# Maaz77/Head-Pose-Estimation-Model

Hardware: AMD Instinct MI355X
Metric: images/sec (train+infer) on 96×96 feature maps; yaw/pitch/roll MAE vs ref (higher is better)
Workload: dtype fp32; 1 GPU; Model-96 create_model(num_filters=360, dropout=0, l2=0.1) training, legacy Adam lr 2.8e-4, 96x96 feature maps (configs[3] per GPU: 512 images per rank); global_batch=512, per_gpu_batch=512, positions_per_image=9216, channels=96, parallelism=dp1

## Files before the change

head-pose-estimation-model_amd/csrc/hpe_mlp2.hip:

```cpp
#include <hip/hip_runtime.h>
#include <stdint.h>
#include <stdlib.h>

#include "hpe_common.h"
#include "hpe_dev.h"

#ifdef MLP2_BIG
#define MLP2_NS mlp2_big
#else
#define MLP2_NS mlp2_small
#endif
#define MLP2_BIG_ROWS (1 << 15)
namespace MLP2_NS {

#define MLP2_MAXW 12
#ifndef MLP2_BAR1_SKIP
#define MLP2_BAR1_SKIP 1
#endif
#ifndef MLP2_W88
#define MLP2_W88 2
#endif
#define MLP2_XS 100
#define MLP2_XF (32 * MLP2_XS)
#define MLP2_LAB 128
#define MLP2_RED 32
#define MLP2_FS 104
#define MLP2_IMG (3 * 32 * MLP2_FS)
#define MLP2_A1W (15 * 68 + 64)
#define MLP2_PRE_HALVES (2 * MLP2_IMG)

struct E2 {
  int act, drop;
  uint32_t thr;
  float keep;
};

struct TileImg {
  int img0, rem0, P;
  template <bool P32 = false>
  __device__ __forceinline__ int of(int r) const {
    const int t = rem0 + r;
    if (P32) return img0 + (t >= P ? 1 : 0);
    return img0 + (P >= 32 ? (t >= P ? 1 : 0) : (P == 1 ? t : t / P));
  }
  __device__ __forceinline__ void advance(int dq, int dr) {
    img0 += dq;
    rem0 += dr;
    if (rem0 >= P) { rem0 -= P; ++img0; }
  }
};

__device__ __forceinline__ float e_fwd(const E2& e, uint64_t seed, int64_t img, int ch, float z) {
  float a = act_f(e.act, z);
  if (e.drop >= 0) a = drop_hash(seed, e.drop, (uint64_t)img, ch) >= e.thr ? a / e.keep : 0.f;
  return a;
}

__device__ __forceinline__ float e_bwd(const E2& e, uint64_t seed, int64_t img, int ch, float g, float val) {
  if (e.drop >= 0) {
    if (drop_hash(seed, e.drop, (uint64_t)img, ch) < e.thr) return 0.f;
    g = g / e.keep;
    val = val * e.keep;
  }
  return e.act == ACT_LINEAR ? g : g * act_grad(e.act, val, 0.f);
}

__device__ __forceinline__ void stage_tile(const Args& args, float* xs, float* lab, int64_t row0,
                                           const TileImg& ti, int wave, int NCB, int lane, int Cin,
                                           bool labels, int XS = MLP2_XS) {
  const int64_t rem = args.nrows - 1 - row0;
  const int last = rem < 31 ? (int)rem : 31;
  const int P = args.P;
  const int q = Cin >> 2;
  if (!args.idx && P >= 32) {
    if (labels && wave == 0) {
#pragma unroll
      for (int pc = 0; pc < 2; ++pc) {
        const int slot = pc * 64 + lane;
        const int r = min(slot >> 2, last), j = min(slot & 3, 2);
        glds4(args.ytrue + (int64_t)ti.of(r) * 3 + j, lds_addr(lab + pc * 64));
      }
    }
    for (int r = wave; r < 32; r += NCB) {
      const int64_t srow = row0 + min(r, last);
      if (lane < q) glds16(args.x + srow * Cin + 4 * lane, lds_addr(xs + r * XS));
    }
    return;
  }
  const int lr = min(lane & 31, last);
  const int limg = ti.of(lr);
  const int lpos = (int)(row0 + lr - (int64_t)limg * P);
  const int lsrc = args.idx ? args.idx[limg] : limg;
  __builtin_amdgcn_s_waitcnt(0x0F70);
  if (labels && wave == 0) {
#pragma unroll
    for (int pc = 0; pc < 2; ++pc) {
      const int slot = pc * 64 + lane;
      const int r = min(slot >> 2, last), j = min(slot & 3, 2);
      const int64_t src = __shfl(lsrc, r, 64);
      glds4(args.ytrue + src * 3 + j, lds_addr(lab + pc * 64));
    }
  }
  for (int r = wave; r < 32; r += NCB) {
    const int rr = min(r, last);
    const int64_t srow = (int64_t)__builtin_amdgcn_readlane(lsrc, rr) * P +
                         __builtin_amdgcn_readlane(lpos, rr);
    if (lane < q) glds16(args.x + srow * Cin + 4 * lane, lds_addr(xs + r * XS));
  }
}

__device__ __forceinline__ int lane_now() {
  int l;
  asm volatile("v_mbcnt_lo_u32_b32 %0, -1, 0\n\tv_mbcnt_hi_u32_b32 %0, -1, %0" : "=v"(l));
  return l;
}

__device__ __forceinline__ void stage_contig(const Args& args, float* xs, float* lab, const float* tp,
                                             int64_t row0, const TileImg& ti, int wave, int NCB, int Cin,
                                             bool labels) {
  const int lane = lane_now();
  const int64_t rem = args.nrows - 1 - row0;
  const int last = rem < 31 ? (int)rem : 31;
  if (labels && wave == 0) {
    const float* yp = args.ytrue + (int64_t)ti.img0 * 3;
#pragma unroll
    for (int pc = 0; pc < 2; ++pc) {
      const int slot = pc * 64 + lane;
      const int r = min(slot >> 2, last), j = min(slot & 3, 2);
      glds4(yp + (ti.rem0 + r >= ti.P ? 3 + j : j), lds_addr(lab + pc * 64));
    }
  }
  const int q = Cin >> 2;
  for (int r = wave; r < 32; r += NCB)
    if (lane < q) glds16(tp + min(r, last) * Cin + 4 * lane, lds_addr(xs + r * MLP2_XS));
}

typedef _Float16 h4 __attribute__((ext_vector_type(4)));

typedef __fp16 fp16x4 __attribute__((__vector_size__(4 * sizeof(__fp16))));

template <int KH>
__device__ __forceinline__ int img_pos(int c) {
  if (KH == 48) return c;
  return c < KH ? c : min(c + 48 - KH, 92);
}
__device__ __forceinline__ h8 tr_read8(const _Float16* p) {
  typedef __attribute__((address_space(3))) fp16x4* lp;
  const fp16x4 a = __builtin_amdgcn_ds_read_tr16_b64_v4f16((lp)(p));
  const fp16x4 b = __builtin_amdgcn_ds_read_tr16_b64_v4f16((lp)(p + 8 * MLP2_FS));
  return __builtin_shufflevector(__builtin_bit_cast(h4, a), __builtin_bit_cast(h4, b), 0, 1, 2, 3, 4, 5, 6, 7);
}
__device__ __forceinline__ constexpr int a1_row(int g) { return 68 * (g ^ ((g >> 1) & 4)); }
#define MLP2_X_LIMIT (65520.f / SPLIT_C)
template <int KH>
__device__ __forceinline__ bool presplit_tile(const float* xs, _Float16* xf, int tid, int NT) {
  bool out = false;
  for (int i = tid; i < 32 * 12; i += NT) {
    const int r = i / 12, rem = i - r * 12, h = rem >= 6 ? 1 : 0, m0 = 8 * (rem - 6 * h);
    const float* s = xs + r * MLP2_XS + KH * h + m0;
    const f32x4 z = {0.f, 0.f, 0.f, 0.f};
    const f32x4 a = *(const f32x4*)(s), b = m0 + 4 < KH ? *(const f32x4*)(s + 4) : z;
    const f32x8 v = {a.x, a.y, a.z, a.w, b.x, b.y, b.z, b.w};
#pragma unroll
    for (int j = 0; j < 8; ++j) out |= !(fabsf(v[j]) < MLP2_X_LIMIT);
    const SplitD d8 = split_d8(v);
    _Float16* d = xf + r * MLP2_FS + 48 * h + m0;
    *(h8*)(d) = d8.ch;
    *(h8*)(d + 32 * MLP2_FS) = d8.cl;
    *(h8*)(d + 64 * MLP2_FS) = d8.h;
  }
  return out;
}

template <int KH, int ACT1, bool DROP, int NWM, bool SPLIT, bool CONTIG = false>
__global__ void __launch_bounds__(NWM * 64) __attribute__((amdgpu_waves_per_eu(NWM == MLP2_MAXW || ACT1 < 0 ? 1 : MLP2_W88, 8))) mlp2_kernel(Args args) {
  static_assert(!CONTIG || (SPLIT && NWM == MLP2_MAXW), "CONTIG is an instantiation of the pre-split kernel");
  if (!SPLIT && args.guard && __hip_atomic_load(args.guard, __ATOMIC_RELAXED, __HIP_MEMORY_SCOPE_AGENT) != args.epoch) return;
#ifdef MLP2_STAMPS
  const uint64_t rt0 = __builtin_amdgcn_s_memrealtime();
#endif
  extern __shared__ __attribute__((aligned(16))) float lds[];
  constexpr int NKB = (2 * KH + 31) / 32;
  constexpr int T = 32;
  constexpr bool PRE = SPLIT && NWM == MLP2_MAXW;
  constexpr int NXB = PRE ? 1 : 2;
  constexpr bool LEAN = PRE && ACT1 >= 0;
  constexpr bool PAD1 = true;
  constexpr int A1S = MLP2_A1W;
  constexpr int HS = NWM == MLP2_MAXW ? 4 : 3;
  const int* prog = args.prog;
  const int* o = prog + prog[H_OPS_OFF];
  const int mode = prog[H_MODE];
  const bool train = mode == MODE_TRAIN;
  const int Cin = o[O_K], F = o[O_N], NCB = o[O_MODE];
  const int wave = __builtin_amdgcn_readfirstlane(threadIdx.x >> 6);
  const int lane = threadIdx.x & 63, half = lane >> 5, l32 = lane & 31;
  const int NT = blockDim.x;
  const int n = wave * 32 + l32;
  const bool nok = n < F;
  const int NPR = NWM == MLP2_MAXW ? MLP2_MAXW : NCB;
  float* xbuf = lds;
  float* lbuf = xbuf + NXB * MLP2_XF;
  float* part = lbuf + 2 * MLP2_LAB;
  float* dz2 = part + NPR * T * 4;
  float* a1s = dz2 + T * 4;
  float* w2t = a1s + NCB * A1S;
  float* b2t = w2t + NCB * 128;
  float* hacc = b2t + 4;
  float* red = hacc + NCB * 64 * HS;
  float* colt = red + MLP2_RED;
  _Float16* xfb = (_Float16*)(colt + NCB * 128);

  E2 e1 = {o[O_EACT], o[O_EDROP], (uint32_t)o[O_ETHR], __int_as_float(o[O_EKEEP])};
  E2 e2 = {o[O_AUX2], o[O_TBASE], (uint32_t)o[O_TCOUNT], __int_as_float(o[O_F0])};
  const float inv_keep1 = 1.f / e1.keep;
  const float* W1 = args.params + o[O_W];
  const float* W2 = args.params + o[O_AUX0];

  const int64_t nrows = args.nrows;
  const int64_t ntiles = (nrows + T - 1) / T;
  const int P = args.P;
  const bool labels = mode != MODE_FWD;
  const int S = gridDim.x * T, dq = S / P, dr = S - dq * P;
  TileImg ti;
  ti.P = P;
  ti.img0 = (int)(blockIdx.x * T / P);
  ti.rem0 = (int)(blockIdx.x * T - ti.img0 * P);
  const float* xnext = CONTIG ? args.x + (int64_t)blockIdx.x * T * Cin : nullptr;
  const int64_t xstep = CONTIG ? (int64_t)gridDim.x * T * Cin : 0;
  if (blockIdx.x < ntiles) {
    if constexpr (CONTIG) stage_contig(args, xbuf, lbuf, xnext, (int64_t)blockIdx.x * T, ti, wave, NCB, Cin, labels);
    else stage_tile(args, xbuf, lbuf, (int64_t)blockIdx.x * T, ti, wave, NCB, lane, Cin, labels);
  }
  xnext += xstep;
  const int nc = min(n, F - 1);
  const float w2a = W2[nc * 3], w2b = W2[nc * 3 + 1], w2c = W2[nc * 3 + 2];
  const int o_bias = __builtin_amdgcn_readfirstlane(o[O_BIAS]), o_aux1 = __builtin_amdgcn_readfirstlane(o[O_AUX1]);
  const float b1r = args.params[max(o_bias, 0) + nc];
  float w2r[2];
#pragma unroll
  for (int t = 0; t < 2; ++t) {
    const int i = threadIdx.x + t * NT, nn = i >> 2, j = i & 3;
    w2r[t] = W2[min(nn, F - 1) * 3 + min(j, 2)];
  }
  const float b2r = args.params[max(o_aux1, 0) + min((int)threadIdx.x & 3, 2)];

  float wreg[SPLIT ? 1 : KH];
  SplitW wsp[SPLIT ? 6 : 1];
  float inv1 = 1.f, s2 = 1.f;
  bool wbad = false;
  if constexpr (SPLIT) {
    f32x8 v[6];
#pragma unroll
    for (int s = 0; s < 6; ++s) {
#pragma unroll
      for (int j = 0; j < 8; ++j) {
        const int k = half * KH + 8 * s + j;
        v[s][j] = 8 * s + j < KH ? W1[(size_t)min(k, Cin - 1) * F + nc] : 0.f;
      }
    }
    __builtin_amdgcn_sched_barrier(0);
    float mx = 0.f;
#pragma unroll
    for (int s = 0; s < 6; ++s) {
#pragma unroll
      for (int j = 0; j < 8; ++j) {
        const int k = half * KH + 8 * s + j;
        v[s][j] = (k < Cin && nok) ? v[s][j] : 0.f;
        mx = fmaxf(mx, fabsf(v[s][j]));
      }
    }
    mx = fmaxf(mx, __shfl_xor(mx, 32, 64));
    const float s1 = pow2_scale(mx, 13);
    inv1 = SPLIT_INV_C / s1;
#pragma unroll
    for (int s = 0; s < 6; ++s) {
      const f32x8 vs = v[s] * s1;
      wsp[s] = split_w8(vs);
      if (PRE) {
#pragma unroll
        for (int j = 0; j < 8; ++j) wbad |= !(fabsf(vs[j]) < 65520.f);
      }
    }
    s2 = pow2_scale(nok ? fmaxf(fmaxf(fabsf(w2a), fabsf(w2b)), fabsf(w2c)) : 0.f, 2);
  } else {
#pragma unroll
    for (int m = 0; m < KH; ++m) {
      const int k = half * KH + m;
      const float wv = W1[(size_t)min(k, Cin - 1) * F + nc];
      wreg[m] = (k < Cin && nok) ? wv : 0.f;
    }
  }
  bool bad = PRE && wbad && blockIdx.x < ntiles;
  {
    const float b1 = (nok && o_bias >= 0) ? b1r : 0.f;
    if (half == 0) *(f32x4*)(colt + n * 4) = f32x4{inv1, b1, s2, 0.f};
  }
#pragma unroll
  for (int t = 0; t < 2; ++t) {
    const int i = threadIdx.x + t * NT, nn = i >> 2, j = i & 3;
    if (i < NCB * 128) w2t[i] = (nn < F && j < 3) ? w2r[t] : 0.f;
  }
  if (threadIdx.x < 4) b2t[threadIdx.x] = (threadIdx.x < 3 && o_aux1 >= 0) ? b2r : 0.f;
  for (int i = threadIdx.x; i < NT * HS; i += NT) hacc[i] = 0.f;

  f32x16 dw[NKB];
#pragma unroll
  for (int s = 0; s < NKB; ++s) dw[s] = f32x16{};
  float dw2[3] = {0.f, 0.f, 0.f};
  float db1 = 0.f;

  const int NT3 = (NT / 3) * 3;

  for (int i = threadIdx.x; i < NXB * 32 * 16; i += NT) {
    const int r = i >> 4, c = Cin + (i & 15);
    if (c < 96) xbuf[r * MLP2_XS + c] = 0.f;
  }
  for (int i = NCB * T * 4 + threadIdx.x; i < NPR * T * 4; i += NT) part[i] = 0.f;
  __syncthreads();
  if constexpr (PRE) {
    asm volatile("s_waitcnt vmcnt(0)" ::: "memory");
    bar_lds();
    const bool xbad = presplit_tile<KH>(xbuf, xfb, threadIdx.x, NT);
    bad |= xbad && blockIdx.x < ntiles;
  }
  int buf = 0;
#ifdef MLP2_STAMPS
  uint32_t ph[9] = {};
  uint64_t tprev = __builtin_amdgcn_s_memtime();
  const uint64_t rt1 = __builtin_amdgcn_s_memrealtime();
#define STAMP(i) do { const uint64_t t_ = __builtin_amdgcn_s_memtime(); ph[i] += (uint32_t)(t_ - tprev); tprev = t_; } while (0)
#else
#define STAMP(i) do {} while (0)
#endif
  for (int tile = blockIdx.x; tile < (int)ntiles; tile += gridDim.x, buf ^= 1, ti.advance(dq, dr)) {
    const int tlane = PRE ? lane_now() : lane, thalf = tlane >> 5, tl32 = tlane & 31;
    const int tcol = wave * 32 + tl32;
    const bool tok = tcol < F;
    const int64_t row0 = (int64_t)tile * T;
    const float* xs = xbuf + (PRE ? 0 : buf) * MLP2_XF;
    const float* lab = lbuf + buf * MLP2_LAB;
    if constexpr (!PRE) asm volatile("s_waitcnt vmcnt(0)" ::: "memory");
    STAMP(0);
    if (!(MLP2_BAR1_SKIP && PRE && tile != (int)blockIdx.x)) bar_lds();
    STAMP(1);
    if (tile + gridDim.x < ntiles) {
      TileImg tn = ti;
      tn.advance(dq, dr);
      if constexpr (CONTIG) {
        stage_contig(args, xbuf, lbuf + (buf ^ 1) * MLP2_LAB, xnext, (int64_t)(tile + gridDim.x) * T, tn,
                     wave, NCB, Cin, labels);
        xnext += xstep;
      } else {
        stage_tile(args, xbuf + (PRE ? 0 : (buf ^ 1)) * MLP2_XF, lbuf + (buf ^ 1) * MLP2_LAB,
                   (int64_t)(tile + gridDim.x) * T, tn, wave, NCB, tlane, Cin, labels);
      }
    }

    STAMP(2);
    uint32_t dmask = 0;
    {
      const float* ap = xs + tl32 * MLP2_XS + thalf * KH;
      f32x16 acc = {};
      if constexpr (PRE) {
        const _Float16* fp = xfb + buf * MLP2_IMG + tl32 * MLP2_FS + 48 * thalf;
        auto frag = [&](int s) {
          return SplitD{*(const h8*)(fp + 8 * s), *(const h8*)(fp + 32 * MLP2_FS + 8 * s),
                        *(const h8*)(fp + 64 * MLP2_FS + 8 * s)};
        };
        SplitD xd = frag(0);
#pragma unroll
        for (int s = 0; s < 6; ++s) {
          SplitD xn = xd;
          if (s + 1 < 6) xn = frag(s + 1);
          __builtin_amdgcn_sched_barrier(0);
          acc = mfma3_dw(xd, wsp[s], acc);
          xd = xn;
        }
        STAMP(3);
      } else if constexpr (SPLIT) {
#pragma unroll
        for (int s = 0; s < 6; ++s) {
          const f32x4 a0 = *(const f32x4*)(ap + 8 * s), a1 = *(const f32x4*)(ap + 8 * s + 4);
          acc = mfma3_dw(split_d8(f32x8{a0.x, a0.y, a0.z, a0.w, a1.x, a1.y, a1.z, a1.w}), wsp[s], acc);
          __builtin_amdgcn_sched_barrier(0);
        }
        bad |= !(fabsf(sum16(acc)) <= 3.0e38f);
      } else {
        f32x4 an = *(const f32x4*)(ap);
#pragma unroll
        for (int m = 0; m < KH; m += 4) {
          const f32x4 a = an;
          if (m + 4 < KH) an = *(const f32x4*)(ap + m + 4);
          acc = __builtin_amdgcn_mfma_f32_32x32x2f32(a.x, wreg[m + 0], acc, 0, 0, 0);
          acc = __builtin_amdgcn_mfma_f32_32x32x2f32(a.y, wreg[m + 1], acc, 0, 0, 0);
          acc = __builtin_amdgcn_mfma_f32_32x32x2f32(a.z, wreg[m + 2], acc, 0, 0, 0);
          acc = __builtin_amdgcn_mfma_f32_32x32x2f32(a.w, wreg[m + 3], acc, 0, 0, 0);
          __builtin_amdgcn_sched_barrier(0);
        }
      }
      if (DROP) {
        if (CONTIG || P >= 32) {
          const bool k0 = drop_hash(args.seed, e1.drop, (uint64_t)(ti.img0 + args.img_off), tcol) >= e1.thr;
          const bool k1 = drop_hash(args.seed, e1.drop, (uint64_t)(ti.img0 + 1 + args.img_off), tcol) >= e1.thr;
#pragma unroll
          for (int g = 0; g < 16; ++g) {
            const int r = (g & 3) + 8 * (g >> 2) + 4 * thalf;
            dmask |= (ti.rem0 + r >= P ? k1 : k0) ? (1u << g) : 0u;
          }
        } else {
#pragma unroll
          for (int g = 0; g < 16; ++g) {
            const int r = (g & 3) + 8 * (g >> 2) + 4 * thalf;
            dmask |= drop_hash(args.seed, e1.drop, (uint64_t)(ti.of(r) + args.img_off), tcol) >= e1.thr
                         ? (1u << g) : 0u;
          }
        }
      }
      const f32x4 cs = *(const f32x4*)(colt + tcol * 4);
#pragma unroll
      for (int g = 0; g < 16; ++g) {
        float z = act1_f<ACT1, SPLIT>(e1.act, SPLIT ? fmaf(acc[g], cs.x, cs.y) : acc[g] + cs.y);
        if (DROP) z = (dmask >> g) & 1u ? z * inv_keep1 : 0.f;
        acc[g] = LEAN || tok ? z : 0.f;
      }
#pragma unroll
      for (int g = 0; g < 16; ++g) a1s[wave * A1S + (PAD1 ? a1_row(g) : 64 * g) + tlane] = acc[g];
      __builtin_amdgcn_fence(__ATOMIC_RELEASE, "wavefront");
      __builtin_amdgcn_wave_barrier();
      __builtin_amdgcn_fence(__ATOMIC_ACQUIRE, "wavefront");
      {
        const int r = tl32, hh = (r >> 2) & 1, gr = (r & 3) + 4 * (r >> 3);
        const float* ar = a1s + wave * A1S + (PAD1 ? a1_row(gr) : 64 * gr) + hh * 32 + 16 * thalf;
        const float* wr = w2t + (wave * 32 + 16 * thalf) * 4;
        float s0 = 0.f, s1 = 0.f, s2 = 0.f;
#pragma unroll
        for (int i = 0; i < 16; i += 4) {
          const f32x4 av = *(const f32x4*)(ar + i);
#pragma unroll
          for (int e = 0; e < 4; ++e) {
            const f32x4 w = *(const f32x4*)(wr + (i + e) * 4);
            s0 = fmaf(av[e], w.x, s0);
            s1 = fmaf(av[e], w.y, s1);
            s2 = fmaf(av[e], w.z, s2);
          }
        }
        s0 += __shfl_xor(s0, 32, 64);
        s1 += __shfl_xor(s1, 32, 64);
        s2 += __shfl_xor(s2, 32, 64);
        if (thalf == 0) *(f32x4*)(part + (wave * T + r) * 4) = f32x4{s0, s1, s2, 0.f};
      }
    }
    STAMP(4);
    if constexpr (PRE) asm volatile("s_waitcnt vmcnt(0)" ::: "memory");
    bar_lds();
    STAMP(5);
    if constexpr (PRE) {
      if (wave >= 2 && tile + gridDim.x < ntiles)
        bad |= presplit_tile<KH>(xbuf, xfb + (buf ^ 1) * MLP2_IMG, threadIdx.x - 128, NT - 128);
    }

    auto head_item = [&](int it) {
      const int r = it / 3, j = it - r * 3;
      const int64_t R = row0 + r;
      float z = b2t[j];
      float pv[MLP2_MAXW];
#pragma unroll
      for (int w = 0; w < MLP2_MAXW; ++w) pv[w] = NWM == MLP2_MAXW || w < NCB ? part[(w * T + r) * 4 + j] : 0.f;
      float lv = 0.f, ha0 = 0.f, ha1 = 0.f, ha2 = 0.f;
      if (mode != MODE_FWD) {
        lv = lab[r * 4 + j];
        ha0 = hacc[threadIdx.x * HS + 0];
        ha1 = hacc[threadIdx.x * HS + 1];
        ha2 = hacc[threadIdx.x * HS + 2];
      }
#pragma unroll
      for (int w = 0; w < MLP2_MAXW; ++w) z += pv[w];
      const bool d2 = ACT1 < 0 || __builtin_expect(e2.drop >= 0, 0);
      int64_t img = 0;
      bool k2 = true;
      if (d2) {
        img = ti.of<CONTIG>(r) + args.img_off;
        if (ACT1 >= 0) k2 = drop_hash(args.seed, e2.drop, (uint64_t)img, j) >= e2.thr;
      }
      const float p = ACT1 >= 0 ? (d2 ? (k2 ? z / e2.keep : 0.f) : z) : e_fwd(e2, args.seed, img, j, z);
      if (mode == MODE_FWD) {
        if (R < nrows) args.y[R * 3 + j] = p;
      } else {
        float g = 0.f;
        if (R < nrows) {
          const float err = p - lv;
          ha0 = fmaf(err, err, ha0);
          ha1 += fabsf(err);
          g = SPLIT ? 2.f * err : 2.f * err * args.inv_count;
        }
        if (train) {
          g = ACT1 >= 0 ? (d2 ? (k2 ? g / e2.keep : 0.f) : g) : e_bwd(e2, args.seed, img, j, g, p);
          dz2[r * 4 + j] = g;
          ha2 += g;
        }
        hacc[threadIdx.x * HS + 0] = ha0;
        hacc[threadIdx.x * HS + 1] = ha1;
        hacc[threadIdx.x * HS + 2] = ha2;
      }
    };
    if constexpr (NWM == MLP2_MAXW) {
      if (threadIdx.x < T * 3) head_item(threadIdx.x);
    } else {
      for (int it = threadIdx.x; it < T * 3 && threadIdx.x < NT3; it += NT3) head_item(it);
    }
    STAMP(6);
    if constexpr (PRE) {
      asm volatile("s_waitcnt vmcnt(0)" ::: "memory");
      bar_lds();
      STAMP(7);
      if (!train) continue;
    } else {
      if (!train) continue;
      bar_lds();
    }

    STAMP(8);
    {
      const f32x4 w2r = *(const f32x4*)(w2t + tcol * 4);
      const float s2 = colt[tcol * 4 + 2];
      const f32x4 w2v = PRE ? f32x4{w2r.x * s2, w2r.y * s2, w2r.z * s2, 0.f} : w2r;
      auto dz_of = [&](int g) {
        const int r = (g & 3) + 8 * (g >> 2) + 4 * thalf;
        const f32x4 d = *(const f32x4*)(dz2 + r * 4);
        const float a = a1s[wave * A1S + (PAD1 ? a1_row(g) : 64 * g) + tlane];
        const float da = PRE ? fmaf(d.z, w2v.z, fmaf(d.x, w2v.x, d.y * w2v.y))
                             : d.x * w2v.x + d.y * w2v.y + d.z * w2v.z;
        float gz, av = a;
        if (DROP) {
          gz = (dmask >> g) & 1u ? da * inv_keep1 : 0.f;
          av = a * e1.keep;
        } else {
          gz = da;
        }
        {
#pragma clang fp contract(off)
          gz = LEAN || tok ? gz * act1_g<ACT1>(e1.act, av) : 0.f;
          db1 += gz;
        }
        dw2[0] = fmaf(a, d.x, dw2[0]);
        dw2[1] = fmaf(a, d.y, dw2[1]);
        dw2[2] = fmaf(a, d.z, dw2[2]);
        return gz;
      };
      if constexpr (PRE) {
        const int tc = (tl32 & 16) + 4 * (tl32 & 3);
        const _Float16* th = xfb + buf * MLP2_IMG + (4 * thalf + ((tl32 >> 2) & 3)) * MLP2_FS;
        auto xt_of = [&](int s, int kb) {
          const _Float16* q = th + 16 * s * MLP2_FS + img_pos<KH>(32 * kb + tc);
          return SplitD{tr_read8(q), tr_read8(q + 32 * MLP2_FS), tr_read8(q + 64 * MLP2_FS)};
        };
        f32x8 dv0, dv1;
#pragma unroll
        for (int j = 0; j < 8; ++j) dv0[j] = dz_of(j);
        const SplitW d0 = split_w8(dv0);
        __builtin_amdgcn_sched_barrier(0);
#pragma unroll
        for (int kb = 0; kb < NKB; ++kb) {
          dw[kb] = mfma3_dw(xt_of(0, kb), d0, dw[kb]);
          if (kb == 0) __builtin_amdgcn_sched_barrier(0);
        }
#pragma unroll
        for (int j = 0; j < 8; ++j) dv1[j] = dz_of(8 + j);
        __builtin_amdgcn_sched_barrier(0);
        const SplitW d1 = split_w8(dv1);
#pragma unroll
        for (int kb = 0; kb < NKB; ++kb) dw[kb] = mfma3_dw(xt_of(1, kb), d1, dw[kb]);
      } else if constexpr (SPLIT) {
#pragma unroll
        for (int s = 0; s < 2; ++s) {
          f32x8 dv;
#pragma unroll
          for (int j = 0; j < 8; ++j) {
            dv[j] = dz_of(8 * s + j);
            if ((j & 3) == 3) __builtin_amdgcn_sched_barrier(0);
          }
          const SplitW dsp = split_w8(dv * s2);
#pragma unroll
          for (int kb = 0; kb < NKB; ++kb) {
            const float* xp = xs + (4 * thalf) * MLP2_XS + kb * 32 + tl32;
            f32x8 xv;
#pragma unroll
            for (int j = 0; j < 8; ++j) xv[j] = xp[(16 * s + 8 * (j >> 2) + (j & 3)) * MLP2_XS];
            dw[kb] = mfma3_dw(split_d8(xv), dsp, dw[kb]);
            __builtin_amdgcn_sched_barrier(0);
          }
        }
      } else {
        float dz1[16];
#pragma unroll
        for (int g = 0; g < 16; ++g) {
          dz1[g] = dz_of(g);
          if ((g & 3) == 3) __builtin_amdgcn_sched_barrier(0);
        }
#pragma unroll
        for (int kb = 0; kb < NKB; ++kb) {
          const float* xp = xs + (4 * thalf) * MLP2_XS + kb * 32 + tl32;
          f32x16 acc = dw[kb];
          auto xat = [&](int g) { return xp[((g & 3) + 8 * (g >> 2)) * MLP2_XS]; };
          float x0 = xat(0), x1 = xat(1);
#pragma unroll
          for (int g = 0; g < 16; ++g) {
            const float xv = x0;
            x0 = x1;
            if (g + 2 < 16) x1 = xat(g + 2);
            acc = __builtin_amdgcn_mfma_f32_32x32x2f32(xv, dz1[g], acc, 0, 0, 0);
            __builtin_amdgcn_sched_barrier(0);
          }
          dw[kb] = acc;
        }
      }
    }
  }

#ifdef MLP2_STAMPS
  const uint64_t rt2 = __builtin_amdgcn_s_memrealtime();
  uint64_t rtA = 0, rtB = 0;
  if (PRE && blockIdx.x == 0 && lane == 0 && (wave == 0 || wave == 5))
    printf("STAMP w%d bwd+tail %u bar1 %u stage %u fwdmfma %u act+part %u bar2 %u head %u bar3 %u presplit %u\n", wave,
           ph[0], ph[1], ph[2], ph[3], ph[4], ph[5], ph[6], ph[7], ph[8]);
#endif
  const int flane = PRE ? lane_now() : lane, fhalf = flane >> 5;
  const int fcol = wave * 32 + (flane & 31);
  const bool fok = fcol < F;
  if (mode == MODE_FWD) {
    if (SPLIT && bad) __hip_atomic_store(args.guard, args.epoch, __ATOMIC_RELAXED, __HIP_MEMORY_SCOPE_AGENT);
    return;
  }
  const int slab = prog[H_SLAB];
  const int npt = prog[H_NPARAMS_TRAIN];
  float* ws = args.ws + (size_t)blockIdx.x * slab;
  const float sc = SPLIT ? args.inv_count : 1.f;
  const int oW = __builtin_amdgcn_readfirstlane(o[O_W]), oB = __builtin_amdgcn_readfirstlane(o[O_BIAS]);
  const int oA0 = __builtin_amdgcn_readfirstlane(o[O_AUX0]), oA1 = __builtin_amdgcn_readfirstlane(o[O_AUX1]);
  __syncthreads();
  const float s2f = colt[fcol * 4 + 2];
  if (train) {
    const float scw = SPLIT ? sc * (SPLIT_INV_C / s2f) : sc;
    float chk = 0.f;
#pragma unroll
    for (int kb = 0; kb < NKB; ++kb) {
      if (SPLIT) chk += sum16(dw[kb]);
#pragma unroll
      for (int g = 0; g < 16; ++g) {
        const int k = kb * 32 + (g & 3) + 8 * (g >> 2) + 4 * fhalf;
        if (k < Cin && fok) ws[oW + (size_t)k * F + fcol] = dw[kb][g] * scw;
      }
    }
    if (SPLIT) bad |= (!LEAN || fok) && !(fabsf(chk) <= 3.0e38f);
    const float tb = (db1 + __shfl_xor(db1, 32, 64)) * (PRE ? 1.f / s2f : 1.f);
    float t2[3];
#pragma unroll
    for (int j = 0; j < 3; ++j) t2[j] = dw2[j] + __shfl_xor(dw2[j], 32, 64);
    if (fhalf == 0 && fok) {
      if (oB >= 0) ws[oB + fcol] = tb * sc;
#pragma unroll
      for (int j = 0; j < 3; ++j) ws[oA0 + fcol * 3 + j] = t2[j] * sc;
    }
#ifdef MLP2_STAMPS
    rtA = __builtin_amdgcn_s_memrealtime();
#endif
    if (oA1 >= 0) {
      for (int j = wave; j < 3; j += NT >> 6) {
        float s = 0.f;
        for (int i = j + 3 * flane; i < NT3; i += 192) s += hacc[i * HS + 2];
        s = wave_sum(s);
        if (flane == 0) ws[oA1 + j] = s * sc;
      }
    }
#ifdef MLP2_STAMPS
    rtB = __builtin_amdgcn_s_memrealtime();
#endif
    __syncthreads();
  }
#ifdef MLP2_STAMPS
  const uint64_t rtC = __builtin_amdgcn_s_memrealtime();
#endif
  if (SPLIT && bad) __hip_atomic_store(args.guard, args.epoch, __ATOMIC_RELAXED, __HIP_MEMORY_SCOPE_AGENT);
  const float a = wave_sum(hacc[threadIdx.x * HS + 0]), b = wave_sum(hacc[threadIdx.x * HS + 1]);
  if (flane == 0) { red[wave] = a; red[MLP2_MAXW + wave] = b; }
  __syncthreads();
  if (threadIdx.x == 0) {
    float s0 = 0.f, s1 = 0.f;
    const int nw = NT >> 6;
    for (int w = 0; w < nw; ++w) { s0 += red[w]; s1 += red[MLP2_MAXW + w]; }
    ws[npt] = s0;
    ws[npt + 1] = s1;
  }
#ifdef MLP2_STAMPS
  if (PRE && threadIdx.x == 0) {
    const uint64_t rt3 = __builtin_amdgcn_s_memrealtime();
    printf("RT wg %d t0 %llu pro %llu loop %llu flush %llu wstore %llu db2 %llu sync %llu tail %llu\n", (int)blockIdx.x, (unsigned long long)rt0,
           (unsigned long long)(rt1 - rt0), (unsigned long long)(rt2 - rt1), (unsigned long long)(rt3 - rt2),
           (unsigned long long)(rtA - rt2), (unsigned long long)(rtB - rtA), (unsigned long long)(rtC - rtB), (unsigned long long)(rt3 - rtC));
  }
#endif
}

#ifdef MLP2_BIG
#define MLP2R_NU 2
#define MLP2R_LDS_FLOATS (2 * MLP2_XF + 2 * MLP2_LAB + MLP2R_NU * MLP2_A1W + 32 * 4 + MLP2R_NU * 128 + 4)

template <int KH, int ACT1, bool DROP>
__global__ void __launch_bounds__(64) __attribute__((amdgpu_waves_per_eu(1, 1))) mlp2r_kernel(Args args) {
  extern __shared__ __attribute__((aligned(16))) float lds[];
  constexpr int NU = MLP2R_NU;
  constexpr int NKB = (2 * KH + 31) / 32;
  constexpr int T = 32;
  constexpr int XS = KH == 44 ? 88 : MLP2_XS;
  const int* prog = args.prog;
  const int* o = prog + prog[H_OPS_OFF];
  const int Cin = o[O_K], F = o[O_N];
  const int lane = threadIdx.x, half = lane >> 5, l32 = lane & 31;
  float* xbuf = lds;
  float* lbuf = xbuf + 2 * MLP2_XF;
  float* a1p = lbuf + 2 * MLP2_LAB;
  float* dz2 = a1p + NU * MLP2_A1W;
  float* w2t = dz2 + 32 * 4;
  float* b2t = w2t + NU * 128;
  const E2 e1 = {o[O_EACT], o[O_EDROP], (uint32_t)o[O_ETHR], __int_as_float(o[O_EKEEP])};
  const E2 e2 = {o[O_AUX2], o[O_TBASE], (uint32_t)o[O_TCOUNT], __int_as_float(o[O_F0])};
  const float inv_keep1 = 1.f / e1.keep, inv_keep2 = 1.f / e2.keep;
  const float* W1 = args.params + o[O_W];
  const float* W2 = args.params + o[O_AUX0];
  const int o_bias = __builtin_amdgcn_readfirstlane(o[O_BIAS]), o_aux1 = __builtin_amdgcn_readfirstlane(o[O_AUX1]);

  const int64_t nrows = args.nrows;
  const int64_t ntiles = (nrows + T - 1) / T;
  const int P = args.P;
  const int S = gridDim.x * T, dq = S / P, dr = S - dq * P;
  TileImg ti;
  ti.P = P;
  ti.img0 = (int)(blockIdx.x * T / P);
  ti.rem0 = (int)(blockIdx.x * T - ti.img0 * P);
  auto stage = [&](float* xd, float* ld, int64_t r0, const TileImg& t) {
    if (XS == 88 && !args.idx && P >= 32 && r0 + T <= nrows && Cin == 88) {
#pragma unroll
      for (int pc = 0; pc < 2; ++pc) {
        const int slot = pc * 64 + lane;
        glds4(args.ytrue + (int64_t)t.of(slot >> 2) * 3 + min(slot & 3, 2), lds_addr(ld + pc * 64));
      }
#pragma unroll
      for (int i = 0; i < 11; ++i) glds16(args.x + r0 * 88 + 256 * i + 4 * lane, lds_addr(xd + 256 * i));
    } else {
      stage_tile(args, xd, ld, r0, t, 0, 1, lane, Cin, true, XS);
    }
  };
  if (blockIdx.x < ntiles) stage(xbuf, lbuf, (int64_t)blockIdx.x * T, ti);

  SplitW wsp[NU][6];
  float inv1[NU], b1v[NU], s2[NU], nm[NU];
  f32x4 w2v[NU];
  bool nok[NU];
  {
    f32x8 v[NU][6];
    float w2r[NU][3], b1r[NU];
#pragma unroll
    for (int u = 0; u < NU; ++u) {
      const int n = 32 * u + l32, nc = min(n, F - 1);
      nok[u] = n < F;
      nm[u] = nok[u] ? 1.f : 0.f;
#pragma unroll
      for (int j = 0; j < 3; ++j) w2r[u][j] = W2[nc * 3 + j];
      b1r[u] = args.params[max(o_bias, 0) + nc];
#pragma unroll
      for (int s = 0; s < 6; ++s) {
#pragma unroll
        for (int j = 0; j < 8; ++j) {
          const int k = half * KH + 8 * s + j;
          v[u][s][j] = 8 * s + j < KH ? W1[(size_t)min(k, Cin - 1) * F + nc] : 0.f;
        }
      }
    }
    const float b2r = args.params[max(o_aux1, 0) + min(lane & 3, 2)];
    __builtin_amdgcn_sched_barrier(0);
#pragma unroll
    for (int u = 0; u < NU; ++u) {
      float mx = 0.f;
#pragma unroll
      for (int s = 0; s < 6; ++s) {
#pragma unroll
        for (int j = 0; j < 8; ++j) {
          const int k = half * KH + 8 * s + j;
          v[u][s][j] = (k < Cin && nok[u]) ? v[u][s][j] : 0.f;
          mx = fmaxf(mx, fabsf(v[u][s][j]));
        }
      }
      mx = fmaxf(mx, __shfl_xor(mx, 32, 64));
      const float s1 = pow2_scale(mx, 13);
      inv1[u] = SPLIT_INV_C / s1;
#pragma unroll
      for (int s = 0; s < 6; ++s) wsp[u][s] = split_w8(v[u][s] * s1);
      w2v[u] = nok[u] ? f32x4{w2r[u][0], w2r[u][1], w2r[u][2], 0.f} : f32x4{0.f, 0.f, 0.f, 0.f};
      s2[u] = pow2_scale(nok[u] ? fmaxf(fmaxf(fabsf(w2r[u][0]), fabsf(w2r[u][1])), fabsf(w2r[u][2])) : 0.f, 2);
      b1v[u] = (nok[u] && o_bias >= 0) ? b1r[u] : 0.f;
      if (half == 0) *(f32x4*)(w2t + (32 * u + l32) * 4) = w2v[u];
    }
    if (lane < 4) b2t[lane] = (lane < 3 && o_aux1 >= 0) ? b2r : 0.f;
  }
  if (XS == 88) {
    for (int i = lane; i < 2 * (MLP2_XF - 32 * 88); i += 64)
      xbuf[(i >= MLP2_XF - 32 * 88 ? MLP2_XF : 0) + 32 * 88 + i % (MLP2_XF - 32 * 88)] = 0.f;
  } else {
    for (int i = lane; i < 2 * 32 * 16; i += 64) {
      const int r = i >> 4, c = Cin + (i & 15);
      if (c < 96) xbuf[r * MLP2_XS + c] = 0.f;
    }
  }

  f32x16 dw[NU][NKB];
#pragma unroll
  for (int u = 0; u < NU; ++u)
#pragma unroll
    for (int kb = 0; kb < NKB; ++kb) dw[u][kb] = f32x16{};
  float dw2[NU][3], db1[NU];
#pragma unroll
  for (int u = 0; u < NU; ++u) { dw2[u][0] = dw2[u][1] = dw2[u][2] = 0.f; db1[u] = 0.f; }
  float sse = 0.f, sae = 0.f, db2[3] = {0.f, 0.f, 0.f};
  bool bad = false;

  int buf = 0;
#ifdef MLP2R_STAMPS
  uint32_t ph[7] = {};
  uint64_t tprev = __builtin_amdgcn_s_memtime();
#define RSTAMP(i) do { const uint64_t t_ = __builtin_amdgcn_s_memtime(); ph[i] += (uint32_t)(t_ - tprev); tprev = t_; } while (0)
#else
#define RSTAMP(i) do {} while (0)
#endif
  for (int64_t tile = blockIdx.x; tile < ntiles; tile += gridDim.x, buf ^= 1, ti.advance(dq, dr)) {
    const int64_t row0 = tile * T;
    RSTAMP(0);
    asm volatile("s_waitcnt vmcnt(0)" ::: "memory");
    if (tile + gridDim.x < ntiles) {
      TileImg tn = ti;
      tn.advance(dq, dr);
      stage(xbuf + (buf ^ 1) * MLP2_XF, lbuf + (buf ^ 1) * MLP2_LAB, (tile + gridDim.x) * T, tn);
    }
    const float* xs = xbuf + buf * MLP2_XF;
    const float* lab = lbuf + buf * MLP2_LAB;
    RSTAMP(1);

    f32x16 acc[NU];
#pragma unroll
    for (int u = 0; u < NU; ++u) acc[u] = f32x16{};
    {
      const float* ap = xs + l32 * XS + half * KH;
      f32x4 xa[12];
#pragma unroll
      for (int s = 0; s < 12; ++s) xa[s] = *(const f32x4*)(ap + 4 * s);
#pragma unroll
      for (int s = 0; s < 6; ++s) {
        const f32x4 a0 = xa[2 * s], a1 = xa[2 * s + 1];
        const SplitD xd = split_d8(f32x8{a0.x, a0.y, a0.z, a0.w, a1.x, a1.y, a1.z, a1.w});
#pragma unroll
        for (int u = 0; u < NU; ++u) acc[u] = mfma3_dw(xd, wsp[u][s], acc[u]);
      }
    }
    RSTAMP(2);
    uint32_t dmask[NU];
#pragma unroll
    for (int u = 0; u < NU; ++u) {
      bad |= !(fabsf(sum16(acc[u])) <= 3.0e38f);
      const int n = 32 * u + l32;
      dmask[u] = 0u;
      if (DROP) {
        if (P >= 32) {
          const bool k0 = drop_hash(args.seed, e1.drop, (uint64_t)(ti.img0 + args.img_off), n) >= e1.thr;
          const bool k1 = drop_hash(args.seed, e1.drop, (uint64_t)(ti.img0 + 1 + args.img_off), n) >= e1.thr;
#pragma unroll
          for (int g = 0; g < 16; ++g) {
            const int r = (g & 3) + 8 * (g >> 2) + 4 * half;
            dmask[u] |= (ti.rem0 + r >= P ? k1 : k0) ? (1u << g) : 0u;
          }
        } else {
#pragma unroll
          for (int g = 0; g < 16; ++g) {
            const int r = (g & 3) + 8 * (g >> 2) + 4 * half;
            dmask[u] |= drop_hash(args.seed, e1.drop, (uint64_t)(ti.of(r) + args.img_off), n) >= e1.thr ? (1u << g) : 0u;
          }
        }
      }
#pragma unroll
      for (int g = 0; g < 16; ++g) {
        const float km = DROP ? ((dmask[u] >> g) & 1u ? inv_keep1 : 0.f) : 1.f;
        acc[u][g] = act1_f<ACT1>(e1.act, fmaf(acc[u][g], inv1[u], b1v[u])) * km * nm[u];
        a1p[u * MLP2_A1W + a1_row(g) + lane] = acc[u][g];
      }
    }
    __builtin_amdgcn_fence(__ATOMIC_RELEASE, "wavefront");
    __builtin_amdgcn_wave_barrier();
    __builtin_amdgcn_fence(__ATOMIC_ACQUIRE, "wavefront");

    RSTAMP(3);
    {
      const int r = l32, hh = (r >> 2) & 1, gr = (r & 3) + 4 * (r >> 3);
      const f32x4 lv = *(const f32x4*)(lab + r * 4);
      float h0 = 0.f, h1 = 0.f, h2 = 0.f;
#pragma unroll
      for (int u = 0; u < NU; ++u) {
        const float* ar = a1p + u * MLP2_A1W + a1_row(gr) + hh * 32 + 16 * half;
        const float* wr = w2t + (32 * u + 16 * half) * 4;
        f32x4 av[4], wv[16];
#pragma unroll
        for (int i = 0; i < 4; ++i) av[i] = *(const f32x4*)(ar + 4 * i);
#pragma unroll
        for (int i = 0; i < 16; ++i) wv[i] = *(const f32x4*)(wr + 4 * i);
#pragma unroll
        for (int i = 0; i < 16; ++i) {
          h0 = fmaf(av[i >> 2][i & 3], wv[i].x, h0);
          h1 = fmaf(av[i >> 2][i & 3], wv[i].y, h1);
          h2 = fmaf(av[i >> 2][i & 3], wv[i].z, h2);
        }
      }
      h0 += __shfl_xor(h0, 32, 64);
      h1 += __shfl_xor(h1, 32, 64);
      h2 += __shfl_xor(h2, 32, 64);
      if (half == 0) {
        const bool valid = row0 + r < nrows;
        const bool d2 = __builtin_expect(e2.drop >= 0, 0);
        const int64_t img = d2 ? ti.of(r) + args.img_off : 0;
        const float zs[3] = {b2t[0] + h0, b2t[1] + h1, b2t[2] + h2};
        float gs[3];
#pragma unroll
        for (int j = 0; j < 3; ++j) {
          const bool k2 = d2 ? drop_hash(args.seed, e2.drop, (uint64_t)img, j) >= e2.thr : true;
          const float kk = d2 ? (k2 ? inv_keep2 : 0.f) : 1.f;
          const float p = zs[j] * kk;
          float g = 0.f;
          if (valid) {
            const float err = p - lv[j];
            sse = fmaf(err, err, sse);
            sae += fabsf(err);
            g = 2.f * err;
          }
          g *= kk;
          db2[j] += g;
          gs[j] = g;
        }
        *(f32x4*)(dz2 + r * 4) = f32x4{gs[0], gs[1], gs[2], 0.f};
      }
    }
    __builtin_amdgcn_fence(__ATOMIC_RELEASE, "wavefront");
    __builtin_amdgcn_wave_barrier();
    __builtin_amdgcn_fence(__ATOMIC_ACQUIRE, "wavefront");

    RSTAMP(4);
    f32x4 dzr[16];
#pragma unroll
    for (int g = 0; g < 16; ++g) dzr[g] = *(const f32x4*)(dz2 + ((g & 3) + 8 * (g >> 2) + 4 * half) * 4);
    f32x8 xtr[2][NKB];
#pragma unroll
    for (int s = 0; s < 2; ++s)
#pragma unroll
      for (int kb = 0; kb < NKB; ++kb)
#pragma unroll
        for (int j = 0; j < 8; ++j)
          xtr[s][kb][j] = xs[(4 * half + 16 * s + 8 * (j >> 2) + (j & 3)) * XS + kb * 32 + l32];
#pragma unroll
    for (int s = 0; s < 2; ++s) {
      f32x8 dv[NU];
#pragma unroll
      for (int j = 0; j < 8; ++j) {
        const int g = 8 * s + j;
        const f32x4 d = dzr[g];
#pragma unroll
        for (int u = 0; u < NU; ++u) {
          const float a = acc[u][g];
          const float da = d.x * w2v[u].x + d.y * w2v[u].y + d.z * w2v[u].z;
          const float km = DROP ? ((dmask[u] >> g) & 1u ? inv_keep1 : 0.f) : 1.f;
          const float gz = da * km * act1_g<ACT1>(e1.act, DROP ? a * e1.keep : a) * nm[u];
          dw2[u][0] = fmaf(a, d.x, dw2[u][0]);
          dw2[u][1] = fmaf(a, d.y, dw2[u][1]);
          dw2[u][2] = fmaf(a, d.z, dw2[u][2]);
          db1[u] += gz;
          dv[u][j] = gz;
        }
      }
      SplitW dsp[NU];
#pragma unroll
      for (int u = 0; u < NU; ++u) dsp[u] = split_w8(dv[u] * s2[u]);
#pragma unroll
      for (int kb = 0; kb < NKB; ++kb) {
        const SplitD xd = split_d8(xtr[s][kb]);
#pragma unroll
        for (int u = 0; u < NU; ++u) dw[u][kb] = mfma3_dw(xd, dsp[u], dw[u][kb]);
      }
      if (s == 0) RSTAMP(5);
    }
    RSTAMP(6);
  }
#ifdef MLP2R_STAMPS
  if (blockIdx.x < 2 && lane == 0)
    printf("RSTAMP wg %d top %u stage %u fwd %u act %u head %u bwd0 %u bwd1 %u\n", (int)blockIdx.x, ph[0], ph[1], ph[2], ph[3], ph[4], ph[5], ph[6]);
#endif

  const int slab = prog[H_SLAB];
  const int npt = prog[H_NPARAMS_TRAIN];
  float* ws = args.ws + (size_t)blockIdx.x * slab;
  const float sc = args.inv_count;
  const int oW = __builtin_amdgcn_readfirstlane(o[O_W]), oA0 = __builtin_amdgcn_readfirstlane(o[O_AUX0]);
  float chk = 0.f;
#pragma unroll
  for (int u = 0; u < NU; ++u) {
    const int n = 32 * u + l32;
    const float scw = sc * (SPLIT_INV_C / s2[u]);
#pragma unroll
    for (int kb = 0; kb < NKB; ++kb) {
      chk += sum16(dw[u][kb]);
#pragma unroll
      for (int g = 0; g < 16; ++g) {
        const int k = kb * 32 + (g & 3) + 8 * (g >> 2) + 4 * half;
        if (k < Cin && nok[u]) ws[oW + (size_t)k * F + n] = dw[u][kb][g] * scw;
      }
    }
    const float tb = db1[u] + __shfl_xor(db1[u], 32, 64);
    float t2[3];
#pragma unroll
    for (int j = 0; j < 3; ++j) t2[j] = dw2[u][j] + __shfl_xor(dw2[u][j], 32, 64);
    if (half == 0 && nok[u]) {
      if (o_bias >= 0) ws[o_bias + n] = tb * sc;
#pragma unroll
      for (int j = 0; j < 3; ++j) ws[oA0 + n * 3 + j] = t2[j] * sc;
    }
  }
  bad |= !(fabsf(chk) <= 3.0e38f);
#pragma unroll
  for (int j = 0; j < 3; ++j) {
    const float t = wave_sum(db2[j]);
    if (lane == 0 && o_aux1 >= 0) ws[o_aux1 + j] = t * sc;
  }
  if (bad) __hip_atomic_store(args.guard, args.epoch, __ATOMIC_RELAXED, __HIP_MEMORY_SCOPE_AGENT);
  const float ta = wave_sum(sse), tb = wave_sum(sae);
  if (lane == 0) {
    ws[npt] = ta;
    ws[npt + 1] = tb;
  }
}
#endif

typedef void (*mlp2_fn)(Args);

template <int KH, bool DROP, int NWM, bool SPLIT, bool CONTIG = false>
static mlp2_fn pick_act(int act, int act2) {
  if (act2 != ACT_LINEAR) return mlp2_kernel<KH, -1, DROP, NWM, SPLIT, CONTIG>;
  if (act == ACT_TANH) return mlp2_kernel<KH, ACT_TANH, DROP, NWM, SPLIT, CONTIG>;
  if (act == ACT_SOFTSIGN) return mlp2_kernel<KH, ACT_SOFTSIGN, DROP, NWM, SPLIT, CONTIG>;
  return mlp2_kernel<KH, -1, DROP, NWM, SPLIT, CONTIG>;
}

template <bool DROP, bool SPLIT>
static mlp2_fn pick_d(int kh, int act, int act2, int ncb, bool contig) {
  if (ncb <= 4) {
    if (kh == 44) return pick_act<44, DROP, 4, SPLIT>(act, act2);
    if (kh == 48) return pick_act<48, DROP, 4, SPLIT>(act, act2);
  }
  if constexpr (SPLIT) {
    if (contig && kh == 44) return pick_act<44, DROP, MLP2_MAXW, SPLIT, true>(act, act2);
    if (contig && kh == 48) return pick_act<48, DROP, MLP2_MAXW, SPLIT, true>(act, act2);
  }
  if (kh == 44) return pick_act<44, DROP, MLP2_MAXW, SPLIT>(act, act2);
  if (kh == 48) return pick_act<48, DROP, MLP2_MAXW, SPLIT>(act, act2);
  return nullptr;
}

static mlp2_fn pick(const int* w, bool split = false, bool contig = false) {
  const int* o = w + w[H_OPS_OFF];
  const int kh = ((o[O_K] + 7) & ~7) / 2, act = o[O_EACT], act2 = o[O_AUX2];
  if (split)
    return o[O_EDROP] >= 0 ? pick_d<true, true>(kh, act, act2, o[O_MODE], contig) : pick_d<false, true>(kh, act, act2, o[O_MODE], contig);
  return o[O_EDROP] >= 0 ? pick_d<true, false>(kh, act, act2, o[O_MODE], false) : pick_d<false, false>(kh, act, act2, o[O_MODE], false);
}

static void geom(const int* w, int& kh, int& rbw, int& ncb, int& lds_bytes, int& act, int& drop) {
  const int* o = w + w[H_OPS_OFF];
  act = o[O_EACT];
  drop = o[O_EDROP];
  const int cin = o[O_K];
  const int cp = (cin + 7) & ~7;
  kh = cp / 2;
  rbw = o[O_FLAGS];
  ncb = o[O_MODE];
  const int T = 32;
  const int npr = ncb > 4 ? MLP2_MAXW : ncb;
  const int rest = 2 * MLP2_LAB + npr * T * 4 + T * 4 + ncb * MLP2_A1W + ncb * 128 + 4 + ncb * 64 * (ncb > 4 ? 4 : 3) + MLP2_RED + ncb * 128;
  lds_bytes = (2 * MLP2_XF + rest) * 4;
  const int pre = (MLP2_XF + rest) * 4 + MLP2_PRE_HALVES * 2;
  if (ncb > 4 && pre > lds_bytes) lds_bytes = pre;
}

static int lds_split(const int* w) {
  int kh, rbw, ncb, lds, act, drop;
  geom(w, kh, rbw, ncb, lds, act, drop);
  return lds;
}

static int launch_k(mlp2_fn k, int nw, int lds, const Args& a, int grid, hipStream_t s) {
  hipFuncSetAttribute((const void*)k, hipFuncAttributeMaxDynamicSharedMemorySize, lds);
  hipLaunchKernelGGL(k, dim3(grid), dim3(nw * 64), lds, s, a);
  return hipGetLastError() == hipSuccess ? 0 : 2;
}

static bool split_only() {
  const char* e = getenv("HPE_SPLIT_ONLY");
  return e && e[0] == '1';
}

#ifdef MLP2_BIG
template <int KH>
static mlp2_fn pick_r_act(int act, bool drop) {
  if (act == ACT_TANH) return drop ? mlp2r_kernel<KH, ACT_TANH, true> : mlp2r_kernel<KH, ACT_TANH, false>;
  if (act == ACT_SOFTSIGN) return drop ? mlp2r_kernel<KH, ACT_SOFTSIGN, true> : mlp2r_kernel<KH, ACT_SOFTSIGN, false>;
  return nullptr;
}
static mlp2_fn pick_r(const int* w) {
  const char* e = getenv("HPE_MLP2_ROWS");
  if ((e && e[0] == '0') || w[H_MODE] != MODE_TRAIN) return nullptr;
  const int* o = w + w[H_OPS_OFF];
  if (o[O_MODE] > MLP2R_NU || o[O_N] > 32 * MLP2R_NU || o[O_AUX2] != ACT_LINEAR) return nullptr;
  const int kh = ((o[O_K] + 7) & ~7) / 2;
  if (kh == 44 && o[O_K] == 88) return pick_r_act<44>(o[O_EACT], o[O_EDROP] >= 0);
  if (kh == 48) return pick_r_act<48>(o[O_EACT], o[O_EDROP] >= 0);
  return nullptr;
}
#else
static mlp2_fn pick_r(const int*) { return nullptr; }
#define MLP2R_LDS_FLOATS 0
#endif

static int launch_pair(const int* w, const Args& a, int grid, hipStream_t s) {
  int kh, rbw, ncb, lds, act, drop;
  geom(w, kh, rbw, ncb, lds, act, drop);
  if (hpe_exact_fp32() || !a.guard) {
    Args e = a;
    e.guard = nullptr;
    const int tv = hpe_tev_begin(s);
    const int rc = launch_k(pick(w), ncb, lds, e, grid, s);
    hpe_tev_end(s, tv);
    return rc;
  }
  const mlp2_fn kr = pick_r(w);
  const int tv = hpe_tev_begin(s);
  const bool contig = a.idx == nullptr && a.P >= 32;
  const int rc = kr ? launch_k(kr, 1, MLP2R_LDS_FLOATS * 4, a, grid, s) : launch_k(pick(w, true, contig), ncb, lds_split(w), a, grid, s);
  hpe_tev_end(s, tv);
  if (rc) return rc;
  if (split_only()) return 0;
  if (a.x_bound > 0.f && a.x_bound < SPLIT_DATA_RANGE) return 0;
  return launch_k(pick(w), ncb, lds, a, grid, s);
}

static int per_cu_of(mlp2_fn k, int ncb, int lds) {
  hipFuncAttributes attr;
  int per_cu = 1;
  if (hipFuncGetAttributes(&attr, (const void*)k) == hipSuccess) {
    const int vg = ((attr.numRegs + 7) / 8) * 8;
    const int waves_simd = vg > 0 ? (512 / vg > 8 ? 8 : 512 / vg) : 8;
    per_cu = (4 * waves_simd) / ncb;
  }
  const int by_lds = (160 * 1024) / lds;
  if (per_cu > by_lds) per_cu = by_lds;
  return per_cu < 1 ? 1 : per_cu;
}

static int cap_per_cu(const int* w) {
  int kh, rbw, ncb, lds, act, drop;
  geom(w, kh, rbw, ncb, lds, act, drop);
  int cap = per_cu_of(pick(w), ncb, lds);
  const int b = per_cu_of(pick(w, true), ncb, lds_split(w)), bc = per_cu_of(pick(w, true, true), ncb, lds_split(w));
  cap = b < cap ? b : cap;
  cap = bc < cap ? bc : cap;
  const mlp2_fn kr = pick_r(w);
  if (kr) {
    const int c = per_cu_of(kr, 1, MLP2R_LDS_FLOATS * 4);
    cap = c < cap ? c : cap;
  }
  return cap;
}
}

#ifdef MLP2_BIG
int mlp2_launch_big(const int* w, const Args& a, int grid, hipStream_t s) {
  return MLP2_NS::launch_pair(w, a, grid, s);
}
int mlp2_per_cu_big(const int* w) { return MLP2_NS::cap_per_cu(w); }
#else
using namespace MLP2_NS;
int mlp2_launch_big(const int* w, const Args& a, int grid, hipStream_t s);
int mlp2_per_cu_big(const int* w);

int mlp2_supported(const int* w) {
  int kh, rbw, ncb, lds, act, drop;
  geom(w, kh, rbw, ncb, lds, act, drop);
  const int* o = w + w[H_OPS_OFF];
  return pick(w) != nullptr && rbw == 1 && ncb >= 1 && ncb <= MLP2_MAXW &&
         o[O_AUX3] == 3 && (o[O_K] & 3) == 0 && o[O_K] <= 96 && lds <= 160 * 1024;
}

int mlp2_grid_cap(const int* w, int n_cu) {
  const int a = MLP2_NS::cap_per_cu(w), b = mlp2_per_cu_big(w);
  return n_cu * (a < b ? a : b);
}

int mlp2_launch(const int* w, const Args& a, int grid, hipStream_t s) {
  if (a.nrows >= MLP2_BIG_ROWS) return mlp2_launch_big(w, a, grid, s);
  return launch_pair(w, a, grid, s);
}
#endif
```

Measured before the change: 187,800 images/sec.

## Fast tanh via exp2/rcp, bpermute xor-shuffles, cheaper split conversion in presplit kernel

Bundles several micro-optimizations in the presplit MLP kernel. Tanh is computed from a native exp2 plus reciprocal, with the 2·log2(e) factor folded into the per-column scale and bias. Half-wave xor shuffles use a raw ds_bpermute keyed on the mbcnt lane id. A lane-derived thread id replaces threadIdx.x in the head, and the dz split conversion uses a cheaper form. A sched_barrier inside the first MFMA loop is also removed. The approximate tanh and split may lose precision, which could affect the MAE checks.

```diff
diff --git a/head-pose-estimation-model_amd/csrc/hpe_mlp2.hip b/head-pose-estimation-model_amd/csrc/hpe_mlp2.hip
--- a/head-pose-estimation-model_amd/csrc/hpe_mlp2.hip
+++ b/head-pose-estimation-model_amd/csrc/hpe_mlp2.hip
@@ -1,6 +1,7 @@
 #include <hip/hip_runtime.h>
 #include <stdint.h>
 #include <stdlib.h>
+#include <type_traits>
 
 #include "hpe_common.h"
 #include "hpe_dev.h"
@@ -113,6 +114,9 @@
   int l;
   asm volatile("v_mbcnt_lo_u32_b32 %0, -1, 0\n\tv_mbcnt_hi_u32_b32 %0, -1, %0" : "=v"(l));
   return l;
+}
+__device__ __forceinline__ float xor32_now(float v, int l) {
+  return __int_as_float(__builtin_amdgcn_ds_bpermute((l ^ 32) << 2, __float_as_int(v)));
 }
 
 __device__ __forceinline__ void stage_contig(const Args& args, float* xs, float* lab, const float* tp,
@@ -172,6 +176,16 @@
   return out;
 }
 
+__device__ __forceinline__ SplitW split_w8_mix(f32x8 v) {
+  SplitW r;
+  r.h = __builtin_convertvector(v, h8);
+  f32x8 lo;
+#pragma unroll
+  for (int j = 0; j < 8; ++j) lo[j] = __builtin_fmaf((float)r.h[j], -SPLIT_C, v[j] * SPLIT_C);
+  r.cl = __builtin_convertvector(lo, h8);
+  return r;
+}
+
 template <int KH, int ACT1, bool DROP, int NWM, bool SPLIT, bool CONTIG = false>
 __global__ void __launch_bounds__(NWM * 64) __attribute__((amdgpu_waves_per_eu(NWM == MLP2_MAXW || ACT1 < 0 ? 1 : MLP2_W88, 8))) mlp2_kernel(Args args) {
   static_assert(!CONTIG || (SPLIT && NWM == MLP2_MAXW), "CONTIG is an instantiation of the pre-split kernel");
@@ -185,6 +199,7 @@
   constexpr bool PRE = SPLIT && NWM == MLP2_MAXW;
   constexpr int NXB = PRE ? 1 : 2;
   constexpr bool LEAN = PRE && ACT1 >= 0;
+  constexpr bool EXPK = PRE && ACT1 == ACT_TANH;
   constexpr bool PAD1 = true;
   constexpr int A1S = MLP2_A1W;
   constexpr int HS = NWM == MLP2_MAXW ? 4 : 3;
@@ -270,7 +285,7 @@
         mx = fmaxf(mx, fabsf(v[s][j]));
       }
     }
-    mx = fmaxf(mx, __shfl_xor(mx, 32, 64));
+    mx = fmaxf(mx, PRE ? xor32_now(mx, lane_now()) : __shfl_xor(mx, 32, 64));
     const float s1 = pow2_scale(mx, 13);
     inv1 = SPLIT_INV_C / s1;
 #pragma unroll
@@ -294,7 +309,8 @@
   bool bad = PRE && wbad && blockIdx.x < ntiles;
   {
     const float b1 = (nok && o_bias >= 0) ? b1r : 0.f;
-    if (half == 0) *(f32x4*)(colt + n * 4) = f32x4{inv1, b1, s2, 0.f};
+    const float ck = EXPK ? 2.8853900817779268f : 1.f;
+    if (half == 0) *(f32x4*)(colt + n * 4) = f32x4{inv1 * ck, b1 * ck, s2, 0.f};
   }
 #pragma unroll
   for (int t = 0; t < 2; ++t) {
@@ -337,6 +353,8 @@
     const int tlane = PRE ? lane_now() : lane, thalf = tlane >> 5, tl32 = tlane & 31;
     const int tcol = wave * 32 + tl32;
     const bool tok = tcol < F;
+    using tid_t = typename std::conditional<PRE, int, unsigned>::type;
+    const tid_t ttid = PRE ? (tid_t)(wave * 64 + tlane) : (tid_t)threadIdx.x;
     const int64_t row0 = (int64_t)tile * T;
     const float* xs = xbuf + (PRE ? 0 : buf) * MLP2_XF;
     const float* lab = lbuf + buf * MLP2_LAB;
@@ -420,7 +438,13 @@
       const f32x4 cs = *(const f32x4*)(colt + tcol * 4);
 #pragma unroll
       for (int g = 0; g < 16; ++g) {
-        float z = act1_f<ACT1, SPLIT>(e1.act, SPLIT ? fmaf(acc[g], cs.x, cs.y) : acc[g] + cs.y);
+        float z;
+        if constexpr (EXPK) {
+          const float e = __builtin_amdgcn_exp2f(fmaf(acc[g], cs.x, cs.y));
+          z = fmaf(-2.f, __builtin_amdgcn_rcpf(1.f + e), 1.f);
+        } else {
+          z = act1_f<ACT1, SPLIT>(e1.act, SPLIT ? fmaf(acc[g], cs.x, cs.y) : acc[g] + cs.y);
+        }
         if (DROP) z = (dmask >> g) & 1u ? z * inv_keep1 : 0.f;
         acc[g] = LEAN || tok ? z : 0.f;
       }
@@ -445,9 +469,15 @@
             s2 = fmaf(av[e], w.z, s2);
           }
         }
-        s0 += __shfl_xor(s0, 32, 64);
-        s1 += __shfl_xor(s1, 32, 64);
-        s2 += __shfl_xor(s2, 32, 64);
+        if constexpr (PRE) {
+          s0 += xor32_now(s0, tlane);
+          s1 += xor32_now(s1, tlane);
+          s2 += xor32_now(s2, tlane);
+        } else {
+          s0 += __shfl_xor(s0, 32, 64);
+          s1 += __shfl_xor(s1, 32, 64);
+          s2 += __shfl_xor(s2, 32, 64);
+        }
         if (thalf == 0) *(f32x4*)(part + (wave * T + r) * 4) = f32x4{s0, s1, s2, 0.f};
       }
     }
@@ -457,7 +487,7 @@
     STAMP(5);
     if constexpr (PRE) {
       if (wave >= 2 && tile + gridDim.x < ntiles)
-        bad |= presplit_tile<KH>(xbuf, xfb + (buf ^ 1) * MLP2_IMG, threadIdx.x - 128, NT - 128);
+        bad |= presplit_tile<KH>(xbuf, xfb + (buf ^ 1) * MLP2_IMG, ttid - 128, NT - 128);
     }
 
     auto head_item = [&](int it) {
@@ -470,9 +500,9 @@
       float lv = 0.f, ha0 = 0.f, ha1 = 0.f, ha2 = 0.f;
       if (mode != MODE_FWD) {
         lv = lab[r * 4 + j];
-        ha0 = hacc[threadIdx.x * HS + 0];
-        ha1 = hacc[threadIdx.x * HS + 1];
-        ha2 = hacc[threadIdx.x * HS + 2];
+        ha0 = hacc[ttid * HS + 0];
+        ha1 = hacc[ttid * HS + 1];
+        ha2 = hacc[ttid * HS + 2];
       }
 #pragma unroll
       for (int w = 0; w < MLP2_MAXW; ++w) z += pv[w];
@@ -499,13 +529,13 @@
           dz2[r * 4 + j] = g;
           ha2 += g;
         }
-        hacc[threadIdx.x * HS + 0] = ha0;
-        hacc[threadIdx.x * HS + 1] = ha1;
-        hacc[threadIdx.x * HS + 2] = ha2;
+        hacc[ttid * HS + 0] = ha0;
+        hacc[ttid * HS + 1] = ha1;
+        hacc[ttid * HS + 2] = ha2;
       }
     };
     if constexpr (NWM == MLP2_MAXW) {
-      if (threadIdx.x < T * 3) head_item(threadIdx.x);
+      if (ttid < T * 3) head_item(ttid);
     } else {
       for (int it = threadIdx.x; it < T * 3 && threadIdx.x < NT3; it += NT3) head_item(it);
     }
@@ -558,17 +588,14 @@
         f32x8 dv0, dv1;
 #pragma unroll
         for (int j = 0; j < 8; ++j) dv0[j] = dz_of(j);
-        const SplitW d0 = split_w8(dv0);
+        const SplitW d0 = split_w8_mix(dv0);
         __builtin_amdgcn_sched_barrier(0);
 #pragma unroll
-        for (int kb = 0; kb < NKB; ++kb) {
-          dw[kb] = mfma3_dw(xt_of(0, kb), d0, dw[kb]);
-          if (kb == 0) __builtin_amdgcn_sched_barrier(0);
-        }
+        for (int kb = 0; kb < NKB; ++kb) dw[kb] = mfma3_dw(xt_of(0, kb), d0, dw[kb]);
 #pragma unroll
         for (int j = 0; j < 8; ++j) dv1[j] = dz_of(8 + j);
         __builtin_amdgcn_sched_barrier(0);
-        const SplitW d1 = split_w8(dv1);
+        const SplitW d1 = split_w8_mix(dv1);
 #pragma unroll
         for (int kb = 0; kb < NKB; ++kb) dw[kb] = mfma3_dw(xt_of(1, kb), d1, dw[kb]);
       } else if constexpr (SPLIT) {
```

Measured after the change: 190,200 images/sec (median of 6 runs). 1.2% higher.
